# AaltoML/SLAM-module

Measured on AMD Instinct MI355X. Metric: frames/sec ORB extract+match (720p), higher is better.
Workload: dtype u8

## Files before the change

include/mi355slam.h:

```cpp
#ifndef MI355SLAM_H
#define MI355SLAM_H

#include <stddef.h>
#include <stdint.h>

#ifdef __cplusplus
extern "C" {
#endif

#define MS_MAX_LEVELS 16
#define MS_ORB_PATCH_RADIUS 19
#define MS_HAMMING_THR_LOW 50
#define MS_HAMMING_THR_HIGH 100
#define MS_HAMMING_MAX 256

typedef enum {
    MS_OK = 0,
    MS_ERR_INVALID = -1,
    MS_ERR_NO_DEVICE = -2,
    MS_ERR_HIP = -3,
    MS_ERR_CAPACITY = -4,
    MS_ERR_NUMERIC = -5,
    MS_ERR_TOO_LATE = -6
} ms_status;
// ... 41 lines not shown
    int32_t max_batch;
    float min_distance;
} ms_orb_config;

typedef struct {
    int32_t capacity;
    int32_t *count;
    float *x, *y;
    float *angle;
    int32_t *octave;
    uint32_t *desc;
    int32_t *track_id;
} ms_keypoints;

int ms_orb_create(ms_ctx *ctx, const ms_orb_config *cfg, ms_orb **out);
void ms_orb_destroy(ms_orb *orb);

int ms_orb_set_valid_mask(ms_orb *orb, const uint8_t *mask_host);

int ms_orb_extract(ms_orb *orb, const uint8_t *images, int images_on_device, int n_frames,
                   size_t frame_stride, size_t row_stride,
                   const float *track_xy, const int32_t *track_id, const int32_t *n_tracks);

int ms_orb_device_view(ms_orb *orb, ms_keypoints *view);
int ms_orb_download(ms_orb *orb, int frame, float *x, float *y, float *angle, int32_t *octave,
                    uint32_t *desc, int32_t *track_id, int32_t *n);
int ms_orb_capacity(const ms_orb *orb);

#define MS_KEYPOINT_RECORD_BYTES 76
int ms_keypoints_pack(ms_ctx *ctx, const ms_keypoints *view, int frame, int n, const double *bearing, uint8_t *records_host);
int ms_keypoints_unpack(const uint8_t *records, int n, float *x, float *y, float *angle, int32_t *octave, double *bearing, uint32_t *desc);

int ms_orb_set_describe_strip(ms_orb *orb, int r);

#define MS_ORB_STAGES 6
int ms_orb_set_profiling(ms_orb *orb, int enable);
int ms_orb_stage_ms(ms_orb *orb, float *ms );
int ms_orb_stage_ms_back(ms_orb *orb, int calls_back, float *ms );
int ms_orb_level_size(const ms_orb *orb, int level, int32_t *w, int32_t *h);
int ms_orb_download_level(ms_orb *orb, int frame, int level, int blurred, uint8_t *dst_host);
int ms_orb_download_detections(ms_orb *orb, int frame, int level, int32_t *x, int32_t *y, int32_t *score, int32_t *n);
int ms_orb_last_candidate_counts(ms_orb *orb, int32_t *out );

int ms_hamming_set_path(ms_ctx *ctx, int path);

int ms_hamming_best2(ms_ctx *ctx, const uint32_t *q, int nq, const uint32_t *t, int nt, int n_pairs,
                     const int32_t *q_bucket, const int32_t *t_bucket, const uint8_t *t_valid,
                     int32_t *best_idx, uint16_t *best_dist, uint16_t *second_dist);

int ms_hamming_best2_sets(ms_ctx *ctx, const uint32_t *q_pool, int q_stride, const int32_t *q_count,
                          const uint32_t *t_pool, int t_stride, const int32_t *t_count,
                          const int32_t *pair_q, const int32_t *pair_t, int n_pairs,
                          int32_t *best_idx, uint16_t *best_dist, uint16_t *second_dist);

int ms_ratio_test(ms_ctx *ctx, const int32_t *best_idx, const uint16_t *best_dist, const uint16_t *second_dist,
                  int n, float lowe_ratio, int max_dist, int32_t *match);

int ms_hamming_candidates(ms_ctx *ctx, const uint32_t *q_desc, int nq, const uint32_t *t_desc,
                          const int32_t *cand_start, const int32_t *cand_idx, const uint8_t *t_skip, const int32_t *t_octave,
                          int32_t *best_idx, uint16_t *best_dist, uint16_t *second_dist, int32_t *best_octave, int32_t *second_octave,
                          int32_t *second_idx );

#define MS_MEDOID_MAX_OBS 256
int ms_descriptor_medoid(ms_ctx *ctx, const uint32_t *desc_pool, const int32_t *obs_start, const int32_t *obs_idx, int n_points,
                         int max_obs, int32_t *best_local, int32_t *best_pool);

// ... 378 lines not shown
```

slam-module_amd/csrc/describe_strips.h:

```cpp
#pragma once
#include <cstdint>

namespace describe_strips {

constexpr int kWaves = 4;
constexpr int kMaxStrip = 8;
constexpr int kMaxRegions = 4;
constexpr int kLongStrip = 4;
constexpr int64_t kGridLimit = 0x7FFFFFFF;

struct Region { int32_t block0, frame0, frames, r, bpf; uint32_t inv; };
struct Plan { Region reg[kMaxRegions]; int32_t regions, blocks; };
struct Strip { int32_t frame, slot0, r; };

constexpr int blocks_per_frame(int capacity, int r) { return (capacity + kWaves * r - 1) / (kWaves * r); }
constexpr int64_t ceil_div(int64_t a, int64_t b) { return (a + b - 1) / b; }

inline bool build(int frames, int capacity, int64_t resident, int forced_r, Plan &out, int long_r = kLongStrip) {
    if (frames < 1 || capacity < 1 || resident < 1 || forced_r < 0 || forced_r > kMaxStrip) return false;
    if (long_r != 2 && long_r != 4 && long_r != 8) return false;
    int r_of[kMaxRegions], n_of[kMaxRegions], n = 0;
    const int64_t bpf1 = blocks_per_frame(capacity, 1);
    if (forced_r > 0) { r_of[0] = forced_r; n_of[0] = frames; n = 1; }
    else if ((int64_t)frames * bpf1 <= 2 * resident) { r_of[0] = 1; n_of[0] = frames; n = 1; }
    else {
        int rest = frames, tail_r[kMaxRegions], tail_n[kMaxRegions], m = 0;
        for (int r = 1; r < long_r && rest > 0; r *= 2) {
            const int64_t want = ceil_div((r == 1 ? 2 : 1) * resident, blocks_per_frame(capacity, r));
            const int take = (int)(want < rest ? want : rest);
            tail_r[m] = r; tail_n[m] = take; ++m; rest -= take;
        }
        if (rest > 0) { r_of[n] = long_r; n_of[n] = rest; ++n; }
        while (m > 0) { --m; r_of[n] = tail_r[m]; n_of[n] = tail_n[m]; ++n; }
    }
    Plan p{};
    int64_t block = 0;
    int frame = 0;
    for (int g = 0; g < kMaxRegions; ++g) {
        if (g < n) {
            const int bpf = blocks_per_frame(capacity, r_of[g]);
            p.reg[g] = Region{(int32_t)block, frame, n_of[g], r_of[g], bpf, 0xFFFFFFFFu / (uint32_t)bpf};
            block += (int64_t)n_of[g] * bpf; frame += n_of[g];
            if (block > kGridLimit) return false;
        } else p.reg[g] = Region{0x7FFFFFFF, frame, 0, 1, 1, 0xFFFFFFFFu};
    }
    p.regions = n; p.blocks = (int32_t)block;
    out = p;
    return true;
}

constexpr Strip decode(const Plan &p, uint32_t block) {
    uint32_t block0 = (uint32_t)p.reg[0].block0, bpf = (uint32_t)p.reg[0].bpf, inv = p.reg[0].inv;
    int32_t frame0 = p.reg[0].frame0, r = p.reg[0].r;
    for (int k = 1; k < kMaxRegions; ++k) {
        const bool in = block >= (uint32_t)p.reg[k].block0;
        block0 = in ? (uint32_t)p.reg[k].block0 : block0; bpf = in ? (uint32_t)p.reg[k].bpf : bpf; inv = in ? p.reg[k].inv : inv;
        frame0 = in ? p.reg[k].frame0 : frame0; r = in ? p.reg[k].r : r;
    }
    const uint32_t local = block - block0;
    uint32_t q = (uint32_t)(((uint64_t)local * inv) >> 32), s = local - q * bpf;
    if (s >= bpf) { ++q; s -= bpf; }
    return Strip{frame0 + (int32_t)q, (int32_t)(s * (uint32_t)(kWaves * r)), r};
}

constexpr int trips(int slot0, int wv, int r, int total) {
    const int t = (total - (slot0 + wv) + kWaves - 1) >> 2;
    return t < 0 ? 0 : (t < r ? t : r);
}

}
```

slam-module_amd/csrc/orb.hip:

```cpp
#include "ms_internal.h"
#include "fast_tiles.h"
#include "describe_strips.h"
#include "describe_lanes.h"
#include "describe_steer.h"
#include "describe_brief_index.h"
#include "resize_vpass.h"
#include <cfloat>
#include <cmath>
#include <cstring>

namespace {

constexpr int kPatchRadius = MS_ORB_PATCH_RADIUS;
using describe_lanes::kHalfPatch;
constexpr int kMaxQuota = 4096;

struct LevelGeom {
    int32_t w, h, pitch, quota;
    int32_t min_dist;
    int32_t det_base;
    int32_t cand_cap;
    int32_t btiles_x, btile_base;
    uint32_t btiles_inv;
    uint64_t img_off, blur_off;
    uint64_t cand_off;
    float scale;
};

struct PyrGeom {
    int32_t levels, lk_level, fast_threshold, max_kpts, max_tracks, capacity;
    int32_t det_stride;
    int32_t width, height, btiles_total, ftiles_total;
    uint64_t slab_stride, cand_stride;
    int32_t umax[16];
// ... 749 lines not shown
    const LevelGeom &G = g->L[g->lk_level];
    int run = 0;
    for (int base = 0; base < n; base += 64) {
        const int i = base + lane;
        bool ok = false; int x = 0, y = 0; float px = 0.f, py = 0.f;
        if (i < n) {
            px = track_xy[((uint64_t)f * g->max_tracks + i) * 2];
            py = track_xy[((uint64_t)f * g->max_tracks + i) * 2 + 1];
            x = __float2int_rn(__fdiv_rn(px, G.scale));
            y = __float2int_rn(__fdiv_rn(py, G.scale));
            ok = x >= kPatchRadius && y >= kPatchRadius && x < G.w - kPatchRadius && y < G.h - kPatchRadius;
            if (ok && valid_mask) {
                const int mx = __float2int_rn(px), my = __float2int_rn(py);
                ok = mx >= 0 && my >= 0 && mx < g->width && my < g->height && valid_mask[(uint64_t)my * g->width + mx] != 0;
            }
        }
        const unsigned long long bal = __ballot(ok);
        if (ok) {
            const uint64_t slot = (uint64_t)f * g->max_tracks + run + __popcll(bal & ((1ull << lane) - 1ull));
            trk_x[slot] = (int16_t)x; trk_y[slot] = (int16_t)y; trk_px[slot] = px; trk_py[slot] = py;
            trk_id[slot] = track_id ? track_id[(uint64_t)f * g->max_tracks + i] : i;
        }
        run += __popcll(bal);
    }
    if (lane == 0) trk_count[f] = run;
}



__device__ __forceinline__ int wave_sum(int v) {
    return __builtin_amdgcn_readlane(wave_scan_add(v), 63);
}

__global__ __launch_bounds__(256) void k_slots(const int16_t *__restrict__ det_x, const int16_t *__restrict__ det_y, const int32_t *__restrict__ det_count,
                                               const int32_t *__restrict__ trk_count, uint2 *__restrict__ slot_tab, int32_t *__restrict__ out_count,
                                               TileLevels TL, int det_stride, int capacity) {
    const int l = blockIdx.x, f = blockIdx.y;
    int base = trk_count[f];
    for (int k = 0; k < l; ++k) base += det_count[f * TL.levels + k];
    const int cnt = det_count[f * TL.levels + l];
    const uint64_t s0 = (uint64_t)f * det_stride + TL.L[l].det_base;
    for (int i = threadIdx.x; i < cnt; i += 256)
        if (base + i < capacity) slot_tab[(uint64_t)f * capacity + base + i] = uint2{(uint32_t)(uint16_t)det_x[s0 + i] | ((uint32_t)(uint16_t)det_y[s0 + i] << 16), (uint32_t)l};
    if (l == TL.levels - 1 && threadIdx.x == 0) out_count[f] = min(base + cnt, capacity);
}


struct DescKp { int x, y, oct, tid_out, pitch, w, h; float ox, oy; bool inner; uint64_t off; };
constexpr int kDescGeoDword = 584, kDescGeoStride = 6, kDescRecDword = kDescGeoDword + kDescGeoStride * MS_MAX_LEVELS, kDescRecStride = 12;
static_assert(kDescRecDword % 4 == 0 && kDescRecDword + kDescRecStride * describe_strips::kMaxStrip <= describe_lanes::kSlabDwords, "per-wave tables fit behind the window");
struct DescRec { uint4 a, b, c; };
__device__ __forceinline__ DescRec desc_read(const uint32_t *rec) {
    return DescRec{*reinterpret_cast<const uint4 *>(rec), *reinterpret_cast<const uint4 *>(rec + 4), *reinterpret_cast<const uint4 *>(rec + 8)};
}
__device__ __forceinline__ DescKp desc_scalars(const DescRec &r) {
    const uint4 a = r.a, b = r.b, c = r.c;
    auto s = [](uint32_t v) { return (uint32_t)__builtin_amdgcn_readfirstlane((int)v); };
    DescKp K;
    K.x = (int)s(a.x); K.y = (int)s(a.y); K.oct = (int)(s(a.z) & 0xFFu); K.inner = (s(a.z) >> 8) != 0; K.tid_out = (int)s(a.w);
    K.ox = __uint_as_float(s(b.x)); K.oy = __uint_as_float(s(b.y)); K.pitch = (int)s(b.z); K.w = (int)s(b.w);
    K.h = (int)s(c.x); K.off = (uint64_t)s(c.y) | ((uint64_t)s(c.z) << 32);
    return K;
}
typedef int v4i_t __attribute__((ext_vector_type(4)));
__device__ __forceinline__ void transpose4_rows(uint32_t (&r)[4]) {
    auto s = __builtin_amdgcn_permlane32_swap(r[0], r[2], false, false); r[0] = s[0]; r[2] = s[1];
    s = __builtin_amdgcn_permlane32_swap(r[1], r[3], false, false); r[1] = s[0]; r[3] = s[1];
    s = __builtin_amdgcn_permlane16_swap(r[0], r[1], false, false); r[0] = s[0]; r[1] = s[1];
    s = __builtin_amdgcn_permlane16_swap(r[2], r[3], false, false); r[2] = s[0]; r[3] = s[1];
}

__global__ __launch_bounds__(256) __attribute__((amdgpu_waves_per_eu(8, 8))) void k_describe(FrameSrc src, TileLevels TL, describe_strips::Plan plan, const uint4 *__restrict__ moment_tab, const float4 *__restrict__ pattern_f,
                                                  const uint2 *__restrict__ slot_tab, int capacity, int max_tracks, int lk_level,
                                                  const int16_t *__restrict__ trk_x, const int16_t *__restrict__ trk_y, const float *__restrict__ trk_px,
                                                  const float *__restrict__ trk_py, const int32_t *__restrict__ trk_id, const int32_t *__restrict__ trk_count,
                                                  float *__restrict__ out_x, float *__restrict__ out_y, float *__restrict__ out_angle,
                                                  int32_t *__restrict__ out_octave, uint32_t *__restrict__ out_desc, int32_t *__restrict__ out_track,
                                                  const int32_t *__restrict__ out_count) {
    const int lane = threadIdx.x & 63, wv = __builtin_amdgcn_readfirstlane(threadIdx.x >> 6);
    const describe_strips::Strip strip = describe_strips::decode(plan, blockIdx.x);
    const int f = strip.frame, R = min(strip.r, describe_strips::kMaxStrip);
    const int slot0 = strip.slot0 + wv;
    __shared__ uint4 s_tab[64 + 256];
    const uint4 tap_v = moment_tab[64 + lane], pair_v = reinterpret_cast<const uint4 *>(pattern_f)[threadIdx.x];
    const uint4 dm = moment_tab[lane];
    const uint32_t dmask[4] = {dm.x, dm.y, dm.z, dm.w};
    const uint32_t wpack_w = reinterpret_cast<const uint32_t *>(moment_tab + 128)[lane];
    __shared__ __attribute__((aligned(16))) uint32_t s_patch[4][describe_lanes::kSlabDwords];
    uint32_t *const win = &s_patch[wv][0], *const geo = win + kDescGeoDword, *const rec = win + kDescRecDword;
    const int total = out_count[f], nt = trk_count[f];
    const uint8_t *const slab_f = src.slab + (uint64_t)f * TL.slab_stride;
    const int myslot = slot0 + 4 * min(lane, R - 1);
    const uint2 ent = slot_tab[(uint64_t)f * capacity + min(myslot, capacity - 1)];
    int tx = 0, ty = 0, tid = -1;
    float tpx = 0.f, tpy = 0.f;
    if (myslot < max_tracks) {
        const uint64_t s2 = (uint64_t)f * max_tracks + myslot;
        tx = trk_x[s2]; ty = trk_y[s2]; tpx = trk_px[s2]; tpy = trk_py[s2]; tid = trk_id[s2];
    }
    const TileLevel &GL = TL.L[lane & (MS_MAX_LEVELS - 1)];
    const int g_pitch = GL.pitch, g_w = GL.w, g_h = GL.h;
    const float g_scale = GL.scale;
    const uint64_t g_off = GL.img_off;
    if (threadIdx.x < 64) s_tab[threadIdx.x] = tap_v;
    s_tab[64 + threadIdx.x] = pair_v;
    if (lane < MS_MAX_LEVELS) {
        const uint64_t off = lane == 0 ? (uint64_t)(uintptr_t)src.lvl0 + (uint64_t)f * src.lvl0_frame_stride - (uint64_t)(uintptr_t)slab_f : g_off;
        uint32_t *g = geo + kDescGeoStride * lane;
        g[0] = (uint32_t)(lane == 0 ? src.lvl0_pitch : g_pitch); g[1] = (uint32_t)g_w; g[2] = (uint32_t)g_h; g[3] = __float_as_uint(g_scale);
        g[4] = (uint32_t)off; g[5] = (uint32_t)(off >> 32);
    }
    __syncthreads();
    const int trips = describe_strips::trips(strip.slot0, wv, R, total);
    if (trips <= 0) return;
    if (lane < R) {
        const bool trk = myslot < nt;
        const int level = trk ? lk_level : (int)min(ent.y, (uint32_t)(MS_MAX_LEVELS - 1));
        const uint32_t *g = geo + kDescGeoStride * level;
        const int pitch = (int)g[0], w = (int)g[1], h = (int)g[2];
        const float scale = __uint_as_float(g[3]);
        const int x = trk ? tx : (int)(ent.x & 0xFFFFu), y = trk ? ty : (int)(ent.x >> 16);
        const float ox = trk ? tpx : __fmul_rn((float)x, scale), oy = trk ? tpy : __fmul_rn((float)y, scale);
        const bool inner = x >= 23 && x + 24 < w && y >= 22 && y + 22 < h;
        const uint64_t off = ((uint64_t)g[4] | ((uint64_t)g[5] << 32)) + (inner ? (uint64_t)((int64_t)(y - 22) * pitch + (x - 23)) : 0ull);
        uint32_t *r = rec + kDescRecStride * lane;
        *reinterpret_cast<uint4 *>(r) = uint4{(uint32_t)x, (uint32_t)y, (uint32_t)level | (inner ? 256u : 0u), (uint32_t)(trk ? tid : -1)};
        *reinterpret_cast<uint4 *>(r + 4) = uint4{__float_as_uint(ox), __float_as_uint(oy), (uint32_t)pitch, (uint32_t)w};
        *reinterpret_cast<uint4 *>(r + 8) = uint4{(uint32_t)h, (uint32_t)off, (uint32_t)(off >> 32), 0u};
    }
    __builtin_amdgcn_fence(__ATOMIC_ACQ_REL, "wavefront");
    __builtin_amdgcn_wave_barrier();
    DescKp K = desc_scalars(desc_read(rec));
    typedef __attribute__((address_space(3))) uint8_t lds_u8_t;
    const uint32_t pbase = (uint32_t)(uintptr_t)(const lds_u8_t *)win + describe_brief_index::kIndexBias;
    const int lane_w = lane;
    __builtin_amdgcn_s_waitcnt(0x0F70);
#pragma unroll 1
    for (int k = 0; k < trips; ++k) {
        int lane_k = lane_w;
        uint32_t wpack = wpack_w;
        asm volatile("" : "+v"(lane_k), "+v"(wpack));
        const int lane = lane_k;
        const int pitch = K.pitch, w = K.w, h = K.h, kx = K.x, ky = K.y;
        uint32_t *pb = win;
        const DescRec next = desc_read(rec + kDescRecStride * min(k + 1, trips - 1));
        if (K.inner) {
            const uint8_t *corner = slab_f + K.off;
            uint32_t off[3];
#pragma unroll
            for (int b = 0; b < 3; ++b) off[b] = __umul24((wpack >> (10 * b)) & 15u, (uint32_t)pitch) + ((wpack >> (10 * b + 4)) & 63u);
#pragma unroll
            for (int t = 0; t < describe_lanes::kWinPieces; ++t) {
                const uint8_t *rows = corner + (uint32_t)(16 * (t / 3)) * (uint32_t)pitch;
                win[lane + 64 * t] = reinterpret_cast<const U32u *>(rows + (describe_lanes::win_active(lane, t) ? off[t % 3] : 0u))->v;
            }
        } else {
            const uint8_t *img = slab_f + K.off;
#pragma unroll 1
            for (int t = 0; t < 9; ++t) {
                const int i = lane + 64 * t, r = i / 12, c = i - 12 * r;
                if (i >= 45 * 12) break;
// ... 46 lines not shown
#pragma unroll
                for (int yt = 0; yt < 3; ++yt) {
                    v4i_t acc = {33024, 33024, 33024, 33024};
                    acc = __builtin_amdgcn_mfma_i32_16x16x64_i8(A2h, Vb[yt], acc, 0, 0, 0);
                    acc <<= 8;
                    acc = __builtin_amdgcn_mfma_i32_16x16x64_i8(A2l, Vb[yt], acc, 0, 0, 0);
                    const int y = 16 * yt + n;
                    if (y < 39 && 4 * t + q < 10)
                        pb[y * 10 + 4 * t + q] = __builtin_amdgcn_perm((uint32_t)acc[1], (uint32_t)acc[0], 0x0C0C0602u) | __builtin_amdgcn_perm((uint32_t)acc[3], (uint32_t)acc[2], 0x06020C0Cu);
                }
            }
        }
        __builtin_amdgcn_fence(__ATOMIC_ACQ_REL, "wavefront");
        __builtin_amdgcn_wave_barrier();
        const float angle_deg = describe_steer::fast_atan2((float)m01, (float)m10);
        const float angle = describe_steer::deg_to_rad(angle_deg);
        const float cs = describe_steer::cos_approx(lane == 1 ? describe_steer::sin_argument(angle) : angle);
        const float ca = __builtin_bit_cast(float, __builtin_amdgcn_readlane(__builtin_bit_cast(int, cs), 0));
        const float sa = __builtin_bit_cast(float, __builtin_amdgcn_readlane(__builtin_bit_cast(int, cs), 1));
        float nsa = -sa;
        asm volatile("" : "+s"(nsa));
        unsigned long long bits[4];
#pragma unroll
        for (int q = 0; q < 4; ++q) {
            const float4 pt = __builtin_bit_cast(float4, s_tab[64 + q * 64 + lane]);
            const float x1 = pt.x, y1 = pt.y, x2 = pt.z, y2 = pt.w;
            const uint32_t r1 = describe_brief_index::round_bits(__fadd_rn(__fmul_rn(x1, sa), __fmul_rn(y1, ca)));
            const uint32_t c1 = describe_brief_index::round_bits(__fadd_rn(__fmul_rn(x1, ca), __fmul_rn(y1, nsa)));
            const uint32_t r2 = describe_brief_index::round_bits(__fadd_rn(__fmul_rn(x2, sa), __fmul_rn(y2, ca)));
            const uint32_t c2 = describe_brief_index::round_bits(__fadd_rn(__fmul_rn(x2, ca), __fmul_rn(y2, nsa)));
            const uint32_t i1 = describe_brief_index::index_from_bits(r1, c1, pbase), i2 = describe_brief_index::index_from_bits(r2, c2, pbase);
            bits[q] = __ballot(*(const lds_u8_t *)(uintptr_t)i1 < *(const lds_u8_t *)(uintptr_t)i2);
        }
        const uint64_t o = (uint64_t)f * capacity + slot0 + 4 * k;
        if (lane < 8) out_desc[o * 8 + lane] = (uint32_t)(bits[lane >> 1] >> ((lane & 1) * 32));
        if (lane == 0) { out_x[o] = K.ox; out_y[o] = K.oy; out_angle[o] = angle_deg; out_octave[o] = K.oct; out_track[o] = K.tid_out; }
        __builtin_amdgcn_fence(__ATOMIC_ACQ_REL, "wavefront");
        __builtin_amdgcn_wave_barrier();
        K = Kn;
    }
}

}

struct ms_orb {
    ms_ctx *ctx = nullptr;
    ms_orb_config cfg{};
    PyrGeom geom{};
    PyrGeom *d_geom = nullptr;
    TileMap blur_tiles{};
    uint2 *d_ftile_tab = nullptr;
    TileLevels tile_levels{};
    uint8_t *d_slab = nullptr;
    uint32_t *d_cand = nullptr;
    int32_t *d_cand_count = nullptr, *d_det_count = nullptr, *d_trk_count = nullptr;
    size_t cand_count_bytes = 0, score_hist_bytes = 0;
    uint32_t *d_score_hist = nullptr;
    int32_t *d_last_count = nullptr;
    int16_t *d_det_x = nullptr, *d_det_y = nullptr, *d_trk_x = nullptr, *d_trk_y = nullptr;
    uint8_t *d_det_score = nullptr, *d_mask = nullptr;
    float *d_trk_px = nullptr, *d_trk_py = nullptr, *d_track_xy = nullptr;
    int32_t *d_trk_id = nullptr, *d_track_id = nullptr, *d_n_tracks = nullptr;
    float *d_x = nullptr, *d_y = nullptr, *d_angle = nullptr;
    int32_t *d_octave = nullptr, *d_track = nullptr, *d_count = nullptr;
    uint2 *d_slot_tab = nullptr;
    uint32_t *d_desc = nullptr;
    int16_t *d_xtab[MS_MAX_LEVELS] = {nullptr}, *d_ytab[MS_MAX_LEVELS] = {nullptr};
    bool wide[MS_MAX_LEVELS] = {false};
    uint4 *d_moment_tab = nullptr;
    float4 *d_pattern_f = nullptr;
    int describe_strip = 0;
    bool profiling = false;
    bool blur_valid = false;
    static constexpr int kProfRing = 128;
    hipEvent_t evr[kProfRing][MS_ORB_STAGES + 1] = {{nullptr}};
    hipEvent_t *ev = evr[0];
    long long prof_calls = 0;
    hipStream_t copy_stream = nullptr;
    hipEvent_t ev_copied[4] = {nullptr}, ev_free[4] = {nullptr}, ev_end = nullptr;
    int chunked_frames = 0;
    bool end_recorded = false;
    FrameSrc last_src{};
    int last_frames = 0;
    bool lvl0_in_slab = false;
    uint64_t lvl0_off = 0;
    int lvl0_pitch = 0;
};

template <typename T>
static int dev_calloc(ms_ctx *c, T **p, size_t n) {
    MS_HIP(c, hipMalloc(reinterpret_cast<void **>(p), n * sizeof(T) ? n * sizeof(T) : 1));
    MS_HIP(c, hipMemsetAsync(*p, 0, n * sizeof(T) ? n * sizeof(T) : 1, c->stream));
    return MS_OK;
}
#define MS_TRY(x) do { int rc__ = (x); if (rc__ != MS_OK) return rc__; } while (0)

__global__ __launch_bounds__(256) void k_pack_keypoints(const float *__restrict__ x, const float *__restrict__ y, const float *__restrict__ angle,
                                                       const int32_t *__restrict__ octave, const uint32_t *__restrict__ desc, const double *__restrict__ bearing,
                                                       uint64_t base, int n, uint32_t *__restrict__ out) {
    const int i = blockIdx.x * 256 + threadIdx.x;
    if (i >= n * 19) return;
    const int k = i / 19, w = i - 19 * k;
    const uint64_t s = base + (uint64_t)k;
// ... 47 lines not shown
        {
            const double su = std::min(w[l], h[l]) / 720.0 * 0.8;
            L.min_dist = (int)std::floor(cfg->min_distance * su + 0.5);
        }
        L.det_base = det_base; det_base += quota[l];
        L.img_off = off; off += (uint64_t)L.pitch * L.h;
        L.blur_off = off; off += (uint64_t)L.pitch * L.h;
        L.cand_cap = (int32_t)ms_align_up((size_t)(((w[l] + 1) / 2) * ((h[l] + 1) / 2) + 256), 4);
        L.cand_off = coff; coff += L.cand_cap;
        L.btiles_x = ms_div_up(w[l], kBlurSeg); L.btile_base = bt; bt += L.btiles_x * ms_div_up(h[l], 4 * kBlurRows);
        L.btiles_inv = (uint32_t)(((1ull << 32) + L.btiles_x - 1) / L.btiles_x);
    }
    G.btiles_total = bt;
    std::vector<uint2> ftab;
    {
        std::vector<fast_tiles::Tile> cover;
        for (int l = 0; l < cfg->levels; ++l) {
            cover.clear();
            fast_tiles::cover(w[l], h[l], cover);
            for (const fast_tiles::Tile &t : cover) ftab.push_back(make_uint2((uint32_t)l | ((uint32_t)t.S << 4), (uint32_t)t.X0 | ((uint32_t)t.Y0 << 16)));
            if (!cover.empty() && (cover.back().X0 > 0xFFFF || cover.back().Y0 > 0xFFFF)) {
                delete o;
                return ms_fail(ctx, MS_ERR_CAPACITY, "ms_orb_create: level %d (%dx%d) is beyond the detector's tile table (65535 px)", l, w[l], h[l]);
            }
        }
    }
    G.ftiles_total = (int)ftab.size();
    if (ftab.size() > 65535) {
        delete o;
        return ms_fail(ctx, MS_ERR_CAPACITY, "ms_orb_create: %zu detector tiles per frame (max 65535)", ftab.size());
    }
    G.det_stride = std::max(cfg->max_kpts, det_base);
    G.capacity = G.det_stride + cfg->max_tracks;
    for (int l = 0; l < cfg->levels; ++l) {
        const LevelGeom &L = G.L[l];
        const int sel_k = (cfg->min_distance > 0.f && L.min_dist >= 2) ? std::min(4 * L.quota, kMaxQuota) : L.quota;
        o->tile_levels.L[l] = TileLevel{L.w, L.h, L.pitch, L.btiles_x, L.cand_cap, L.btiles_inv, L.img_off, L.blur_off, L.cand_off, L.scale, L.det_base, sel_k};
    }
    for (int l = 0; l <= MS_MAX_LEVELS; ++l) o->blur_tiles.base[l] = l < cfg->levels ? G.L[l].btile_base : bt;
    G.slab_stride = ms_align_up(off, 256); G.cand_stride = coff;
    o->tile_levels.slab_stride = G.slab_stride; o->tile_levels.cand_stride = G.cand_stride; o->tile_levels.levels = G.levels; o->tile_levels.fast_threshold = G.fast_threshold;
    o->lvl0_off = G.L[0].img_off; o->lvl0_pitch = G.L[0].pitch;
    const size_t B = cfg->max_batch, cap = G.capacity;
    int rc = MS_OK;
    auto A = [&](int r) { if (rc == MS_OK) rc = r; };
    A(dev_calloc(ctx, &o->d_geom, 1));
    A(dev_calloc(ctx, &o->d_slab, B * G.slab_stride + 256));
    A(dev_calloc(ctx, &o->d_cand, B * G.cand_stride));
    A(dev_calloc(ctx, &o->d_cand_count, B * MS_MAX_LEVELS));
    o->cand_count_bytes = sizeof(int32_t) * B * MS_MAX_LEVELS;
    A(dev_calloc(ctx, &o->d_score_hist, B * MS_MAX_LEVELS * 256));
    o->score_hist_bytes = sizeof(uint32_t) * B * MS_MAX_LEVELS * 256;
    A(dev_calloc(ctx, &o->d_last_count, B * MS_MAX_LEVELS));
    A(dev_calloc(ctx, &o->d_det_count, B * MS_MAX_LEVELS));
    A(dev_calloc(ctx, &o->d_trk_count, B));
    A(dev_calloc(ctx, &o->d_det_x, B * (size_t)G.det_stride));
    A(dev_calloc(ctx, &o->d_det_y, B * (size_t)G.det_stride));
    A(dev_calloc(ctx, &o->d_det_score, B * (size_t)G.det_stride));
    const size_t T = (size_t)std::max(cfg->max_tracks, 1);
    A(dev_calloc(ctx, &o->d_trk_x, B * T)); A(dev_calloc(ctx, &o->d_trk_y, B * T));
    A(dev_calloc(ctx, &o->d_trk_px, B * T)); A(dev_calloc(ctx, &o->d_trk_py, B * T));
    A(dev_calloc(ctx, &o->d_trk_id, B * T)); A(dev_calloc(ctx, &o->d_track_xy, B * T * 2));
    A(dev_calloc(ctx, &o->d_track_id, B * T)); A(dev_calloc(ctx, &o->d_n_tracks, B));
    A(dev_calloc(ctx, &o->d_x, B * cap)); A(dev_calloc(ctx, &o->d_y, B * cap)); A(dev_calloc(ctx, &o->d_angle, B * cap));
    A(dev_calloc(ctx, &o->d_octave, B * cap)); A(dev_calloc(ctx, &o->d_track, B * cap)); A(dev_calloc(ctx, &o->d_count, B)); A(dev_calloc(ctx, &o->d_slot_tab, B * cap));
    A(dev_calloc(ctx, &o->d_desc, B * cap * 8));
// ... 53 lines not shown
}

void ms_orb_destroy(ms_orb *o) {
    if (!o) return;
    (void)hipSetDevice(o->ctx->device);
    (void)hipStreamSynchronize(o->ctx->stream);
    void *ptrs[] = {o->d_geom, o->d_slab, o->d_cand, o->d_cand_count, o->d_score_hist, o->d_last_count, o->d_det_count, o->d_trk_count, o->d_det_x, o->d_det_y,
                    o->d_det_score, o->d_mask, o->d_trk_x, o->d_trk_y, o->d_trk_px, o->d_trk_py, o->d_trk_id, o->d_track_xy,
                    o->d_track_id, o->d_n_tracks, o->d_x, o->d_y, o->d_angle, o->d_octave, o->d_track, o->d_count, o->d_desc, o->d_slot_tab};
    for (void *p : ptrs) if (p) (void)hipFree(p);
    if (o->d_moment_tab) (void)hipFree(o->d_moment_tab);
    if (o->d_pattern_f) (void)hipFree(o->d_pattern_f);
    if (o->d_ftile_tab) (void)hipFree(o->d_ftile_tab);
    for (auto &set : o->evr) for (int i = 0; i <= MS_ORB_STAGES; ++i) if (set[i]) (void)hipEventDestroy(set[i]);
    if (o->copy_stream) { (void)hipStreamSynchronize(o->copy_stream); (void)hipStreamDestroy(o->copy_stream); }
    for (int i = 0; i < 4; ++i) { if (o->ev_copied[i]) (void)hipEventDestroy(o->ev_copied[i]); if (o->ev_free[i]) (void)hipEventDestroy(o->ev_free[i]); }
    if (o->ev_end) (void)hipEventDestroy(o->ev_end);

    for (int l = 0; l < MS_MAX_LEVELS; ++l) {
        if (o->d_xtab[l]) (void)hipFree(o->d_xtab[l]);
        if (o->d_ytab[l]) (void)hipFree(o->d_ytab[l]);
    }
    delete o;
}

int ms_orb_capacity(const ms_orb *o) { return o ? o->geom.capacity : MS_ERR_INVALID; }

int ms_orb_set_describe_strip(ms_orb *o, int r) {
    if (!o || r < 0 || r > describe_strips::kMaxStrip) return MS_ERR_INVALID;
    o->describe_strip = r;
    return MS_OK;
}

int ms_orb_set_profiling(ms_orb *o, int enable) {
    if (!o) return MS_ERR_INVALID;
    ms_ctx *c = o->ctx;
    if (enable && !o->evr[0][0])
        for (auto &set : o->evr) for (int i = 0; i <= MS_ORB_STAGES; ++i) MS_HIP(c, hipEventCreate(&set[i]));
    o->profiling = enable != 0;
    return MS_OK;
}

int ms_orb_stage_ms_back(ms_orb *o, int calls_back, float *ms) {
    if (!o || !ms || calls_back < 0 || calls_back >= ms_orb::kProfRing) return MS_ERR_INVALID;
    ms_ctx *c = o->ctx;
    if (!o->evr[0][0] || calls_back >= o->prof_calls) return ms_fail(c, MS_ERR_INVALID, "ms_orb_stage_ms_back: no profiled call %d calls back", calls_back);
    hipEvent_t *set = o->evr[(o->prof_calls - 1 - calls_back) % ms_orb::kProfRing];
    MS_HIP(c, hipEventSynchronize(set[MS_ORB_STAGES]));
    for (int i = 0; i < MS_ORB_STAGES; ++i) MS_HIP(c, hipEventElapsedTime(&ms[i], set[i], set[i + 1]));
    return MS_OK;
}

int ms_orb_stage_ms(ms_orb *o, float *ms) {
    if (!o || !ms) return MS_ERR_INVALID;
    ms_ctx *c = o->ctx;
    if (!o->profiling || o->last_frames == 0) return ms_fail(c, MS_ERR_INVALID, "ms_orb_stage_ms: profiling is off or nothing ran");
    MS_HIP(c, hipEventSynchronize(o->ev[MS_ORB_STAGES]));
    for (int i = 0; i < MS_ORB_STAGES; ++i) MS_HIP(c, hipEventElapsedTime(&ms[i], o->ev[i], o->ev[i + 1]));
    return MS_OK;
}

int ms_orb_set_valid_mask(ms_orb *o, const uint8_t *mask) {
    if (!o) return MS_ERR_INVALID;
    ms_ctx *c = o->ctx;
    MS_HIP(c, hipStreamSynchronize(c->stream));
    if (!mask) { if (o->d_mask) { MS_HIP(c, hipFree(o->d_mask)); o->d_mask = nullptr; } return MS_OK; }
// ... 48 lines not shown
        MS_KERNEL_CHECK(c, "k_resize");
    }
    pyramid_range.end();
    MS_STAGE_MARK();
    o->blur_valid = false;
    MS_STAGE_MARK();
    MsRange detect_range("detect");
    counters_dirty = true;
    if (prune) hipLaunchKernelGGL(k_fast<true>, dim3(nf, G.ftiles_total), dim3(kFastThreads), 0, st, src, cand, cand_count, score_hist, o->d_ftile_tab, o->tile_levels);
    else hipLaunchKernelGGL(k_fast<false>, dim3(G.ftiles_total, nf), dim3(kFastThreads), 0, st, src, cand, cand_count, score_hist, o->d_ftile_tab, o->tile_levels);
    MS_KERNEL_CHECK(c, "k_fast");
    MS_STAGE_MARK();
    const bool few = nf * G.levels <= 64;
    if (o->cfg.min_distance > 0.f) {
        if (few) hipLaunchKernelGGL((k_select<true, 1024>), dim3(G.levels, nf), dim3(1024), 0, st, o->d_geom, cand, cand_count, o->d_mask, det_x, det_y, det_score, det_count, score_hist, last_count);
        else hipLaunchKernelGGL((k_select<true, 256>), dim3(G.levels, nf), dim3(256), 0, st, o->d_geom, cand, cand_count, o->d_mask, det_x, det_y, det_score, det_count, score_hist, last_count);
    } else {
        if (few) hipLaunchKernelGGL((k_select<false, 1024>), dim3(G.levels, nf), dim3(1024), 0, st, o->d_geom, cand, cand_count, o->d_mask, det_x, det_y, det_score, det_count, score_hist, last_count);
        else hipLaunchKernelGGL((k_select<false, 256>), dim3(G.levels, nf), dim3(256), 0, st, o->d_geom, cand, cand_count, o->d_mask, det_x, det_y, det_score, det_count, score_hist, last_count);
    }
    MS_KERNEL_CHECK(c, "k_select");
    counters_dirty = false;
    MS_STAGE_MARK();
    if (o->cfg.max_tracks > 0) {
        hipLaunchKernelGGL(k_tracks, dim3(nf), dim3(64), 0, st, o->d_geom, have_tracks ? o->d_track_xy + F * T * 2 : nullptr,
                           (have_tracks && have_ids) ? o->d_track_id + F * T : nullptr, have_tracks ? o->d_n_tracks + F : nullptr, o->d_mask,
                           o->d_trk_x + F * T, o->d_trk_y + F * T, o->d_trk_px + F * T, o->d_trk_py + F * T, o->d_trk_id + F * T, trk_count);
        MS_KERNEL_CHECK(c, "k_tracks");
    }
    MS_STAGE_MARK();
    detect_range.end();
    MsRange describe_range("describe");
    const size_t C = (size_t)G.capacity;
    hipLaunchKernelGGL(k_slots, dim3(G.levels, nf), dim3(256), 0, st, det_x, det_y, det_count, trk_count, o->d_slot_tab + F * C, o->d_count + F, o->tile_levels, G.det_stride, G.capacity);
    MS_KERNEL_CHECK(c, "k_slots");
    describe_strips::Plan plan;
    if (!describe_strips::build(nf, G.capacity, 8ll * std::max(c->n_cu, 1), o->describe_strip, plan)) return ms_fail(c, MS_ERR_CAPACITY, "k_describe: %d frames of %d slots exceed the grid", nf, G.capacity);
    hipLaunchKernelGGL(k_describe, dim3(plan.blocks), dim3(256), 0, st, src, o->tile_levels, plan, o->d_moment_tab, o->d_pattern_f,
                       o->d_slot_tab + F * C, G.capacity, G.max_tracks, G.lk_level, o->d_trk_x + F * T, o->d_trk_y + F * T, o->d_trk_px + F * T, o->d_trk_py + F * T, o->d_trk_id + F * T, trk_count, o->d_x + F * C, o->d_y + F * C,
                       o->d_angle + F * C, o->d_octave + F * C, o->d_desc + F * C * 8, o->d_track + F * C, o->d_count + F);
    MS_KERNEL_CHECK(c, "k_describe");
    MS_STAGE_MARK();
#undef MS_STAGE_MARK
    return MS_OK;
}

static int orb_extract_enqueue(ms_orb *o, const uint8_t *images, int on_device, int n_frames, size_t frame_stride, size_t row_stride,
                               const float *track_xy, const int32_t *track_id, const int32_t *n_tracks, bool &counters_dirty) {
    ms_ctx *c = o->ctx;
    const PyrGeom &G = o->geom;
    if (n_frames < 1 || n_frames > o->cfg.max_batch) return ms_fail(c, MS_ERR_CAPACITY, "ms_orb_extract: n_frames %d outside [1,%d]", n_frames, o->cfg.max_batch);
    if (row_stride < (size_t)G.width || frame_stride < row_stride * (size_t)(G.height - 1) + G.width)
        return ms_fail(c, MS_ERR_INVALID, "ms_orb_extract: strides smaller than the frame");
    MS_HIP(c, hipSetDevice(c->device));
    hipStream_t st = c->stream;
    MS_TRY(ms_ctx_order_after_downloads(c));
    FrameSrc src{};
    src.slab = o->d_slab;
    const bool have_tracks = track_xy && n_tracks && o->cfg.max_tracks > 0;
    if (have_tracks) {
        const size_t T = o->cfg.max_tracks;
        MS_HIP(c, hipMemcpyAsync(o->d_track_xy, track_xy, (size_t)n_frames * T * 2 * sizeof(float), hipMemcpyHostToDevice, st));
        MS_HIP(c, hipMemcpyAsync(o->d_n_tracks, n_tracks, (size_t)n_frames * sizeof(int32_t), hipMemcpyHostToDevice, st));
        if (track_id) MS_HIP(c, hipMemcpyAsync(o->d_track_id, track_id, (size_t)n_frames * T * sizeof(int32_t), hipMemcpyHostToDevice, st));
    }
    const bool aligned = on_device && (reinterpret_cast<uintptr_t>(images) % 16 == 0) && (row_stride % 16 == 0) && (frame_stride % 16 == 0);
    if (aligned) {
        src.lvl0 = images; src.lvl0_frame_stride = frame_stride; src.lvl0_pitch = (int)row_stride;
        o->lvl0_in_slab = false;
        MS_TRY(orb_enqueue_kernels(o, src, 0, n_frames, have_tracks, track_id != nullptr, counters_dirty));
    } else {
        uint8_t *dst = o->d_slab + o->lvl0_off;
// ... 166 lines not shown
```

slam-module_amd/mi355slam/__init__.py:

```python
import ctypes as C
import os
import weakref

import numpy as np

_HERE = os.path.dirname(os.path.abspath(__file__))
LIB_PATH = os.path.join(os.path.dirname(_HERE), "lib", "libmi355slam.so")
MAX_LEVELS = 16

u8p = C.POINTER(C.c_uint8)
i32p = C.POINTER(C.c_int32)
u32p = C.POINTER(C.c_uint32)
u16p = C.POINTER(C.c_uint16)
f32p = C.POINTER(C.c_float)
f64p = C.POINTER(C.c_double)


class MsError(RuntimeError):
    pass


class OrbConfig(C.Structure):
    _fields_ = [("width", C.c_int32), ("height", C.c_int32), ("levels", C.c_int32), ("scale_factor", C.c_float),
                ("max_kpts", C.c_int32), ("lk_track_level", C.c_int32), ("fast_threshold", C.c_int32),
# ... 248 lines not shown
                    txy[f, :k] = np.asarray(track_xy[f], np.float32).reshape(k, 2)
                    tid[f, :k] = np.asarray(track_id[f], np.int32) if track_id is not None else np.arange(k)
        self.ctx.check(lib().ms_orb_extract(self._h, _vp(images), on_device, n_frames, C.c_size_t(frame_stride),
                                            C.c_size_t(row_stride), _vp(txy), _vp(tid), _vp(nt)), "ms_orb_extract")
        self.n_frames = n_frames

    def device_view(self):
        v = KeypointsView()
        self.ctx.check(lib().ms_orb_device_view(self._h, C.byref(v)), "ms_orb_device_view")
        return v

    def download(self, frame):
        cap = self.capacity
        out = dict(x=np.zeros(cap, np.float32), y=np.zeros(cap, np.float32), angle=np.zeros(cap, np.float32),
                   octave=np.zeros(cap, np.int32), desc=np.zeros((cap, 8), np.uint32), track_id=np.zeros(cap, np.int32))
        n = C.c_int32()
        self.ctx.check(lib().ms_orb_download(self._h, frame, _vp(out["x"]), _vp(out["y"]), _vp(out["angle"]), _vp(out["octave"]),
                                             _vp(out["desc"]), _vp(out["track_id"]), C.byref(n)), "ms_orb_download")
        return {k: v[:n.value].copy() for k, v in out.items()}

    def pack_keypoints(self, frame, bearing=None):
        self.ctx.sync()
        v = self.device_view()
        cnt = np.zeros(1, np.int32)
        self.ctx.check(lib().ms_dev_download(self.ctx._h, _vp(cnt), C.c_void_p(v.count + 4 * frame), C.c_size_t(4)), "ms_dev_download")
        n = int(cnt[0])
        out = np.zeros((n, 76), np.uint8)
        db = None if bearing is None else self.ctx.upload(np.ascontiguousarray(bearing, np.float64).reshape(n, 3))
        self.ctx.check(lib().ms_keypoints_pack(self.ctx._h, C.byref(v), frame, n, _vp(db), _vp(out)), "ms_keypoints_pack")
        return out

    def set_describe_strip(self, r):
        self.ctx.check(lib().ms_orb_set_describe_strip(self._h, int(r)), "ms_orb_set_describe_strip")

    def set_profiling(self, enable=True):
        self.ctx.check(lib().ms_orb_set_profiling(self._h, int(enable)), "ms_orb_set_profiling")

    def stage_ms(self):
        ms = (C.c_float * 6)()
        self.ctx.check(lib().ms_orb_stage_ms(self._h, ms), "ms_orb_stage_ms")
        return dict(zip(("resize", "blur", "fast", "select", "tracks", "describe"), [float(v) for v in ms]))

    def stage_ms_back(self, calls_back):
        ms = (C.c_float * 6)()
        self.ctx.check(lib().ms_orb_stage_ms_back(self._h, int(calls_back), ms), "ms_orb_stage_ms_back")
        return dict(zip(("resize", "blur", "fast", "select", "tracks", "describe"), [float(v) for v in ms]))

    def level_size(self, level):
        w, h = C.c_int32(), C.c_int32()
        self.ctx.check(lib().ms_orb_level_size(self._h, level, C.byref(w), C.byref(h)), "ms_orb_level_size")
        return w.value, h.value

    def download_level(self, frame, level, blurred=False):
        w, h = self.level_size(level)
        out = np.zeros((h, w), np.uint8)
        self.ctx.check(lib().ms_orb_download_level(self._h, frame, level, int(blurred), _vp(out)), "ms_orb_download_level")
        return out

    def download_detections(self, frame, level):
        q = self.capacity
        x, y, s = np.zeros(q, np.int32), np.zeros(q, np.int32), np.zeros(q, np.int32)
        n = C.c_int32()
        self.ctx.check(lib().ms_orb_download_detections(self._h, frame, level, _vp(x), _vp(y), _vp(s), C.byref(n)), "ms_orb_download_detections")
        return x[:n.value].copy(), y[:n.value].copy(), s[:n.value].copy()

    def last_candidate_counts(self):
# ... 1185 lines not shown
```

Baseline: 173,100.

## Remap describe blocks per XCD and add optional spatial keypoint ordering

Adds a block-index remap in the describe kernel so that consecutive strips of a region land on the same XCD, to improve L2 locality of image reads across the chiplets. Adds an optional serpentine band sort of keypoints in k_slots, off by default, which carries the original output slot through the slot table so descriptors still land in their fixed positions. The long strip length also grows from 4 to 8. Costs are extra index arithmetic per block, a capacity limit from packing the slot into 24 bits, and a possibly less balanced grid.

```diff
diff --git a/include/mi355slam.h b/include/mi355slam.h
--- a/include/mi355slam.h
+++ b/include/mi355slam.h
@@ -97,6 +97,8 @@
 int ms_keypoints_unpack(const uint8_t *records, int n, float *x, float *y, float *angle, int32_t *octave, double *bearing, uint32_t *desc);
 
 int ms_orb_set_describe_strip(ms_orb *orb, int r);
+
+int ms_orb_set_describe_order(ms_orb *orb, int mode);
 
 #define MS_ORB_STAGES 6
 int ms_orb_set_profiling(ms_orb *orb, int enable);
diff --git a/slam-module_amd/csrc/describe_order.h b/slam-module_amd/csrc/describe_order.h
--- /dev/null
+++ b/slam-module_amd/csrc/describe_order.h
@@ -0,0 +1,30 @@
+#pragma once
+#include <cstdint>
+
+namespace describe_order {
+
+constexpr int kRemap = 1;
+constexpr int kSpatial = 2;
+constexpr int kModeMask = kRemap | kSpatial;
+constexpr int kDefaultMode = kRemap;
+
+constexpr int kBandShift = 5, kBandRows = 1 << kBandShift;
+constexpr int kCoordBits = 15, kIndexBits = 12;
+
+constexpr int kMaxBands = 1 << (kCoordBits - kBandShift);
+constexpr uint32_t band_of(int y) { return (uint32_t)y >> kBandShift; }
+constexpr uint32_t in_band_key(int x, uint32_t band, int index) {
+    const uint32_t along = (band & 1u) ? (uint32_t)((1 << kCoordBits) - 1 - x) : (uint32_t)x;
+    return (along << kIndexBits) | (uint32_t)index;
+}
+constexpr uint64_t key(int x, int y, int index) {
+    return ((uint64_t)band_of(y) << (kCoordBits + kIndexBits)) | in_band_key(x, band_of(y), index);
+}
+constexpr int index_of(uint64_t k) { return (int)(k & ((1u << kIndexBits) - 1)); }
+
+constexpr int kSlotShift = 8;
+constexpr uint32_t pack(int level, int slot) { return (uint32_t)level | ((uint32_t)slot << kSlotShift); }
+constexpr int level_of(uint32_t e) { return (int)(e & ((1u << kSlotShift) - 1)); }
+constexpr int slot_of(uint32_t e) { return (int)(e >> kSlotShift); }
+
+}
diff --git a/slam-module_amd/csrc/describe_strips.h b/slam-module_amd/csrc/describe_strips.h
--- a/slam-module_amd/csrc/describe_strips.h
+++ b/slam-module_amd/csrc/describe_strips.h
@@ -6,7 +6,7 @@
 constexpr int kWaves = 4;
 constexpr int kMaxStrip = 8;
 constexpr int kMaxRegions = 4;
-constexpr int kLongStrip = 4;
+constexpr int kLongStrip = 8;
 constexpr int64_t kGridLimit = 0x7FFFFFFF;
 
 struct Region { int32_t block0, frame0, frames, r, bpf; uint32_t inv; };
@@ -63,6 +63,22 @@
     return Strip{frame0 + (int32_t)q, (int32_t)(s * (uint32_t)(kWaves * r)), r};
 }
 
+constexpr int kXcds = 8;
+constexpr uint32_t remap(const Plan &p, uint32_t block) {
+    uint32_t block0 = (uint32_t)p.reg[0].block0, end = (uint32_t)p.reg[1].block0;
+    for (int k = 1; k < kMaxRegions; ++k) {
+        const bool in = block >= (uint32_t)p.reg[k].block0;
+        block0 = in ? (uint32_t)p.reg[k].block0 : block0;
+        const uint32_t next = k + 1 < kMaxRegions ? (uint32_t)p.reg[k + 1 < kMaxRegions ? k + 1 : k].block0 : (uint32_t)p.blocks;
+        end = in ? next : end;
+    }
+    end = end < (uint32_t)p.blocks ? end : (uint32_t)p.blocks;
+    const uint32_t local = block - block0, n = end - block0;
+    const uint32_t x = local % kXcds, j = local / kXcds, q = n / kXcds, rem = n % kXcds;
+    const uint32_t start = x < rem ? x * (q + 1) : rem * (q + 1) + (x - rem) * q;
+    return block0 + start + j;
+}
+
 constexpr int trips(int slot0, int wv, int r, int total) {
     const int t = (total - (slot0 + wv) + kWaves - 1) >> 2;
     return t < 0 ? 0 : (t < r ? t : r);
diff --git a/slam-module_amd/csrc/orb.hip b/slam-module_amd/csrc/orb.hip
--- a/slam-module_amd/csrc/orb.hip
+++ b/slam-module_amd/csrc/orb.hip
@@ -1,5 +1,6 @@
 #include "ms_internal.h"
 #include "fast_tiles.h"
+#include "describe_order.h"
 #include "describe_strips.h"
 #include "describe_lanes.h"
 #include "describe_steer.h"
@@ -815,21 +816,62 @@
     return __builtin_amdgcn_readlane(wave_scan_add(v), 63);
 }
 
+template <bool SPATIAL>
 __global__ __launch_bounds__(256) void k_slots(const int16_t *__restrict__ det_x, const int16_t *__restrict__ det_y, const int32_t *__restrict__ det_count,
                                                const int32_t *__restrict__ trk_count, uint2 *__restrict__ slot_tab, int32_t *__restrict__ out_count,
                                                TileLevels TL, int det_stride, int capacity) {
-    const int l = blockIdx.x, f = blockIdx.y;
+    __shared__ uint32_t s_key[SPATIAL ? kMaxQuota : 1];
+    __shared__ uint16_t s_y[SPATIAL ? kMaxQuota : 1];
+    __shared__ int s_start[SPATIAL ? describe_order::kMaxBands : 1], s_cur[SPATIAL ? describe_order::kMaxBands : 1], s_w[4];
+    const int l = blockIdx.x, f = blockIdx.y, tid = threadIdx.x;
     int base = trk_count[f];
     for (int k = 0; k < l; ++k) base += det_count[f * TL.levels + k];
     const int cnt = det_count[f * TL.levels + l];
+    const int n = max(min(min(cnt, capacity - base), kMaxQuota), 0);
     const uint64_t s0 = (uint64_t)f * det_stride + TL.L[l].det_base;
-    for (int i = threadIdx.x; i < cnt; i += 256)
-        if (base + i < capacity) slot_tab[(uint64_t)f * capacity + base + i] = uint2{(uint32_t)(uint16_t)det_x[s0 + i] | ((uint32_t)(uint16_t)det_y[s0 + i] << 16), (uint32_t)l};
-    if (l == TL.levels - 1 && threadIdx.x == 0) out_count[f] = min(base + cnt, capacity);
-}
-
-
-struct DescKp { int x, y, oct, tid_out, pitch, w, h; float ox, oy; bool inner; uint64_t off; };
+    uint2 *const tab = slot_tab + (uint64_t)f * capacity + base;
+    if constexpr (!SPATIAL) {
+        for (int i = tid; i < n; i += 256) tab[i] = uint2{(uint32_t)(uint16_t)det_x[s0 + i] | ((uint32_t)(uint16_t)det_y[s0 + i] << 16), describe_order::pack(l, base + i)};
+    } else {
+        for (int b = tid; b < describe_order::kMaxBands; b += 256) s_cur[b] = 0;
+        __syncthreads();
+        for (int i = tid; i < n; i += 256) atomicAdd(&s_cur[min(describe_order::band_of(det_y[s0 + i] & 0x7FFF), (uint32_t)describe_order::kMaxBands - 1)], 1);
+        __syncthreads();
+        {
+            int c[4], sum = 0;
+#pragma unroll
+            for (int k = 0; k < 4; ++k) { c[k] = s_cur[4 * tid + k]; sum += c[k]; }
+            const int incl = wave_scan_add(sum);
+            if ((tid & 63) == 63) s_w[tid >> 6] = incl;
+            __syncthreads();
+            int at = incl - sum;
+            for (int w = 0; w < (tid >> 6); ++w) at += s_w[w];
+#pragma unroll
+            for (int k = 0; k < 4; ++k) { s_start[4 * tid + k] = at; s_cur[4 * tid + k] = at; at += c[k]; }
+        }
+        __syncthreads();
+        for (int i = tid; i < n; i += 256) {
+            const int x = det_x[s0 + i] & 0x7FFF, y = det_y[s0 + i] & 0x7FFF;
+            const uint32_t band = describe_order::band_of(y);
+            const int p = atomicAdd(&s_cur[band], 1);
+            s_key[p] = describe_order::in_band_key(x, band, i); s_y[p] = (uint16_t)y;
+        }
+        __syncthreads();
+        for (int p = tid; p < n; p += 256) {
+            const uint32_t mine = s_key[p], y = s_y[p], band = describe_order::band_of((int)y);
+            const int lo = s_start[band], hi = s_cur[band];
+            int pos = lo;
+            for (int q = lo; q < hi; ++q) pos += s_key[q] < mine;
+            const int i = (int)(mine & ((1u << describe_order::kIndexBits) - 1));
+            const uint32_t along = mine >> describe_order::kIndexBits, x = (band & 1u) ? (uint32_t)((1 << describe_order::kCoordBits) - 1) - along : along;
+            tab[pos] = uint2{x | (y << 16), describe_order::pack(l, base + i)};
+        }
+    }
+    if (l == TL.levels - 1 && tid == 0) out_count[f] = min(base + cnt, capacity);
+}
+
+
+struct DescKp { int x, y, oct, tid_out, pitch, w, h, slot; float ox, oy; bool inner; uint64_t off; };
 constexpr int kDescGeoDword = 584, kDescGeoStride = 6, kDescRecDword = kDescGeoDword + kDescGeoStride * MS_MAX_LEVELS, kDescRecStride = 12;
 static_assert(kDescRecDword % 4 == 0 && kDescRecDword + kDescRecStride * describe_strips::kMaxStrip <= describe_lanes::kSlabDwords, "per-wave tables fit behind the window");
 struct DescRec { uint4 a, b, c; };
@@ -842,7 +884,7 @@
     DescKp K;
     K.x = (int)s(a.x); K.y = (int)s(a.y); K.oct = (int)(s(a.z) & 0xFFu); K.inner = (s(a.z) >> 8) != 0; K.tid_out = (int)s(a.w);
     K.ox = __uint_as_float(s(b.x)); K.oy = __uint_as_float(s(b.y)); K.pitch = (int)s(b.z); K.w = (int)s(b.w);
-    K.h = (int)s(c.x); K.off = (uint64_t)s(c.y) | ((uint64_t)s(c.z) << 32);
+    K.h = (int)s(c.x); K.off = (uint64_t)s(c.y) | ((uint64_t)s(c.z) << 32); K.slot = (int)s(c.w);
     return K;
 }
 typedef int v4i_t __attribute__((ext_vector_type(4)));
@@ -854,14 +896,14 @@
 }
 
 __global__ __launch_bounds__(256) __attribute__((amdgpu_waves_per_eu(8, 8))) void k_describe(FrameSrc src, TileLevels TL, describe_strips::Plan plan, const uint4 *__restrict__ moment_tab, const float4 *__restrict__ pattern_f,
-                                                  const uint2 *__restrict__ slot_tab, int capacity, int max_tracks, int lk_level,
+                                                  const uint2 *__restrict__ slot_tab, int capacity, int max_tracks, int lk_level, int xcd_runs,
                                                   const int16_t *__restrict__ trk_x, const int16_t *__restrict__ trk_y, const float *__restrict__ trk_px,
                                                   const float *__restrict__ trk_py, const int32_t *__restrict__ trk_id, const int32_t *__restrict__ trk_count,
                                                   float *__restrict__ out_x, float *__restrict__ out_y, float *__restrict__ out_angle,
                                                   int32_t *__restrict__ out_octave, uint32_t *__restrict__ out_desc, int32_t *__restrict__ out_track,
                                                   const int32_t *__restrict__ out_count) {
     const int lane = threadIdx.x & 63, wv = __builtin_amdgcn_readfirstlane(threadIdx.x >> 6);
-    const describe_strips::Strip strip = describe_strips::decode(plan, blockIdx.x);
+    const describe_strips::Strip strip = describe_strips::decode(plan, xcd_runs ? describe_strips::remap(plan, blockIdx.x) : blockIdx.x);
     const int f = strip.frame, R = min(strip.r, describe_strips::kMaxStrip);
     const int slot0 = strip.slot0 + wv;
     __shared__ uint4 s_tab[64 + 256];
@@ -898,7 +940,7 @@
     if (trips <= 0) return;
     if (lane < R) {
         const bool trk = myslot < nt;
-        const int level = trk ? lk_level : (int)min(ent.y, (uint32_t)(MS_MAX_LEVELS - 1));
+        const int level = trk ? lk_level : min(describe_order::level_of(ent.y), MS_MAX_LEVELS - 1);
         const uint32_t *g = geo + kDescGeoStride * level;
         const int pitch = (int)g[0], w = (int)g[1], h = (int)g[2];
         const float scale = __uint_as_float(g[3]);
@@ -909,7 +951,7 @@
         uint32_t *r = rec + kDescRecStride * lane;
         *reinterpret_cast<uint4 *>(r) = uint4{(uint32_t)x, (uint32_t)y, (uint32_t)level | (inner ? 256u : 0u), (uint32_t)(trk ? tid : -1)};
         *reinterpret_cast<uint4 *>(r + 4) = uint4{__float_as_uint(ox), __float_as_uint(oy), (uint32_t)pitch, (uint32_t)w};
-        *reinterpret_cast<uint4 *>(r + 8) = uint4{(uint32_t)h, (uint32_t)off, (uint32_t)(off >> 32), 0u};
+        *reinterpret_cast<uint4 *>(r + 8) = uint4{(uint32_t)h, (uint32_t)off, (uint32_t)(off >> 32), (uint32_t)(trk ? myslot : describe_order::slot_of(ent.y))};
     }
     __builtin_amdgcn_fence(__ATOMIC_ACQ_REL, "wavefront");
     __builtin_amdgcn_wave_barrier();
@@ -1022,7 +1064,7 @@
             const uint32_t i1 = describe_brief_index::index_from_bits(r1, c1, pbase), i2 = describe_brief_index::index_from_bits(r2, c2, pbase);
             bits[q] = __ballot(*(const lds_u8_t *)(uintptr_t)i1 < *(const lds_u8_t *)(uintptr_t)i2);
         }
-        const uint64_t o = (uint64_t)f * capacity + slot0 + 4 * k;
+        const uint64_t o = (uint64_t)f * capacity + K.slot;
         if (lane < 8) out_desc[o * 8 + lane] = (uint32_t)(bits[lane >> 1] >> ((lane & 1) * 32));
         if (lane == 0) { out_x[o] = K.ox; out_y[o] = K.oy; out_angle[o] = angle_deg; out_octave[o] = K.oct; out_track[o] = K.tid_out; }
         __builtin_amdgcn_fence(__ATOMIC_ACQ_REL, "wavefront");
@@ -1059,6 +1101,7 @@
     bool wide[MS_MAX_LEVELS] = {false};
     uint4 *d_moment_tab = nullptr;
     float4 *d_pattern_f = nullptr;
+    int describe_order = describe_order::kDefaultMode;
     int describe_strip = 0;
     bool profiling = false;
     bool blur_valid = false;
@@ -1172,6 +1215,10 @@
     }
     G.det_stride = std::max(cfg->max_kpts, det_base);
     G.capacity = G.det_stride + cfg->max_tracks;
+    if (G.capacity >= (1 << (32 - describe_order::kSlotShift))) {
+        delete o;
+        return ms_fail(ctx, MS_ERR_CAPACITY, "ms_orb_create: %d output slots per frame (max %d)", G.capacity, (1 << (32 - describe_order::kSlotShift)) - 1);
+    }
     for (int l = 0; l < cfg->levels; ++l) {
         const LevelGeom &L = G.L[l];
         const int sel_k = (cfg->min_distance > 0.f && L.min_dist >= 2) ? std::min(4 * L.quota, kMaxQuota) : L.quota;
@@ -1291,6 +1338,12 @@
     return MS_OK;
 }
 
+int ms_orb_set_describe_order(ms_orb *o, int mode) {
+    if (!o || mode < 0 || (mode & ~describe_order::kModeMask)) return MS_ERR_INVALID;
+    o->describe_order = mode;
+    return MS_OK;
+}
+
 int ms_orb_set_profiling(ms_orb *o, int enable) {
     if (!o) return MS_ERR_INVALID;
     ms_ctx *c = o->ctx;
@@ -1405,12 +1458,15 @@
     detect_range.end();
     MsRange describe_range("describe");
     const size_t C = (size_t)G.capacity;
-    hipLaunchKernelGGL(k_slots, dim3(G.levels, nf), dim3(256), 0, st, det_x, det_y, det_count, trk_count, o->d_slot_tab + F * C, o->d_count + F, o->tile_levels, G.det_stride, G.capacity);
+    if (o->describe_order & describe_order::kSpatial)
+        hipLaunchKernelGGL(k_slots<true>, dim3(G.levels, nf), dim3(256), 0, st, det_x, det_y, det_count, trk_count, o->d_slot_tab + F * C, o->d_count + F, o->tile_levels, G.det_stride, G.capacity);
+    else
+        hipLaunchKernelGGL(k_slots<false>, dim3(G.levels, nf), dim3(256), 0, st, det_x, det_y, det_count, trk_count, o->d_slot_tab + F * C, o->d_count + F, o->tile_levels, G.det_stride, G.capacity);
     MS_KERNEL_CHECK(c, "k_slots");
     describe_strips::Plan plan;
     if (!describe_strips::build(nf, G.capacity, 8ll * std::max(c->n_cu, 1), o->describe_strip, plan)) return ms_fail(c, MS_ERR_CAPACITY, "k_describe: %d frames of %d slots exceed the grid", nf, G.capacity);
     hipLaunchKernelGGL(k_describe, dim3(plan.blocks), dim3(256), 0, st, src, o->tile_levels, plan, o->d_moment_tab, o->d_pattern_f,
-                       o->d_slot_tab + F * C, G.capacity, G.max_tracks, G.lk_level, o->d_trk_x + F * T, o->d_trk_y + F * T, o->d_trk_px + F * T, o->d_trk_py + F * T, o->d_trk_id + F * T, trk_count, o->d_x + F * C, o->d_y + F * C,
+                       o->d_slot_tab + F * C, G.capacity, G.max_tracks, G.lk_level, o->describe_order & describe_order::kRemap, o->d_trk_x + F * T, o->d_trk_y + F * T, o->d_trk_px + F * T, o->d_trk_py + F * T, o->d_trk_id + F * T, trk_count, o->d_x + F * C, o->d_y + F * C,
                        o->d_angle + F * C, o->d_octave + F * C, o->d_desc + F * C * 8, o->d_track + F * C, o->d_count + F);
     MS_KERNEL_CHECK(c, "k_describe");
     MS_STAGE_MARK();
diff --git a/slam-module_amd/mi355slam/__init__.py b/slam-module_amd/mi355slam/__init__.py
--- a/slam-module_amd/mi355slam/__init__.py
+++ b/slam-module_amd/mi355slam/__init__.py
@@ -304,6 +304,9 @@
 
     def set_describe_strip(self, r):
         self.ctx.check(lib().ms_orb_set_describe_strip(self._h, int(r)), "ms_orb_set_describe_strip")
+
+    def set_describe_order(self, mode):
+        self.ctx.check(lib().ms_orb_set_describe_order(self._h, int(mode)), "ms_orb_set_describe_order")
 
     def set_profiling(self, enable=True):
         self.ctx.check(lib().ms_orb_set_profiling(self._h, int(enable)), "ms_orb_set_profiling")
```

Result: faster. 175,700, median of 6 (+1.5%).
